# lightbulb128/troy-nova

Hardware: AMD Instinct MI355X
Metric: homomorphic mul+relinearize ops/sec (CKKS mul+relin+rescale), N=16384 (higher is better)
Workload: dtype u64; 1 GPU; CKKS N=16384, 6x50-bit coeff modulus (K=6, L=5): multiply + relinearize + rescale_to_next (BASELINE configs[2]); batch_per_gpu=1024, entry=troyn_ckks_multiply_relinearize_rescale, parallelism=batch-sharded x1, keys broadcast once (RCCL), ranks=1, slowest_rank=0

## Files before the change

### troy-nova_amd/csrc/launch.hpp

```cpp
#pragma once
#include <hip/hip_runtime.h>
#include "ntt_kernels.hpp"
#include "ntt_sizes.hpp"
#include "ksmac_kernels.hpp"
#include "behz2_kernels.hpp"

#ifndef TROYN_SMALL_LP_FACTOR
#define TROYN_SMALL_LP_FACTOR 2
#endif

namespace troyn {

inline unsigned device_cu_count() {
    static thread_local int cached_dev = -1;
    static thread_local unsigned cached = 0;
    int dev = 0;
    (void)hipGetDevice(&dev);
    if (dev != cached_dev) {
        int cus = 0;
        if (hipDeviceGetAttribute(&cus, hipDeviceAttributeMultiprocessorCount, dev) != hipSuccess || cus <= 0) cus = 256;
        cached = (unsigned)cus; cached_dev = dev;
    }
    return cached;
}
inline bool is_small_launch(size_t limb_polys) { return limb_polys * TROYN_SMALL_LP_FACTOR <= device_cu_count(); }

struct LaunchCtx {
    hipStream_t s;
    int half_mask;
    bool small_two_pass_off;
    int tensor_wgs;
};

template <class A, int PART>
struct NttUnit {
    static bool transform(unsigned log_n, const NttArgs& a, size_t limb_polys, bool inverse, const LaunchCtx& lc, u64* scratch);
    static bool small_pass(unsigned log_n, int which, const NttArgs& a, size_t limb_polys, const LaunchCtx& lc);
    static bool ks_mac(unsigned log_n, const NttArgs& a, const KeyPtrs& kp, size_t blocks, const LaunchCtx& lc);
    static bool tensor(unsigned log_n, int stage, const NttArgs& a, const NttArgs& b, const NttArgs& d, size_t batch, const LaunchCtx& lc);
};
extern template struct NttUnit<ArithF64, 1>;
extern template struct NttUnit<ArithF64, 2>;
extern template struct NttUnit<ArithU64, 1>;
extern template struct NttUnit<ArithU64, 2>;
template <class F>
inline bool in_ntt_unit(unsigned log_n, bool f64, F&& f) {
    if (ntt_part_of(log_n) == 1) return f64 ? f(NttUnit<ArithF64, 1>{}) : f(NttUnit<ArithU64, 1>{});
    return f64 ? f(NttUnit<ArithF64, 2>{}) : f(NttUnit<ArithU64, 2>{});
}

inline bool launch_transform(unsigned log_n, bool f64, const NttArgs& a, size_t limb_polys, bool inverse, const LaunchCtx& lc, u64* scratch) {
    return in_ntt_unit(log_n, f64, [&](auto u) { return decltype(u)::transform(log_n, a, limb_polys, inverse, lc, scratch); });
}
void launch_ntt_generic(const NttArgs& a, unsigned log_n, bool inverse, size_t limb_polys, const LaunchCtx& lc);
inline bool launch_small_pass(unsigned log_n, bool f64, int which, const NttArgs& a, size_t limb_polys, const LaunchCtx& lc) {
    return in_ntt_unit(log_n, f64, [&](auto u) { return decltype(u)::small_pass(log_n, which, a, limb_polys, lc); });
}
void launch_mrr_quartet(unsigned log_n, size_t batch, const NttArgs& sp, const NttArgs& la, const NttArgs& ta, hipStream_t s, bool limb_parallel);
void launch_mrr_quartet_load(unsigned log_n, size_t groups, const NttArgs& iv, const NttArgs& fw, hipStream_t s, bool f64);
void launch_mrr_tail(unsigned log_n, size_t batch, const NttArgs& sp, const NttArgs& la, const NttArgs& ta, hipStream_t s);
inline bool launch_ks_mac(unsigned log_n, bool f64, const NttArgs& a, const KeyPtrs& kp, size_t blocks, const LaunchCtx& lc) {
    return in_ntt_unit(log_n, f64, [&](auto u) { return decltype(u)::ks_mac(log_n, a, kp, blocks, lc); });
}
inline bool launch_tensor(unsigned log_n, bool f64, int stage, const NttArgs& a, const NttArgs& b, const NttArgs& d, size_t batch, const LaunchCtx& lc) {
    return in_ntt_unit(log_n, f64, [&](auto u) { return decltype(u)::tensor(log_n, stage, a, b, d, batch, lc); });
}
bool launch_tensor_accumulate(unsigned log_n, bool f64, const NttArgs& fa, const TensorAccPtrs& terms, unsigned count, const NttArgs& id, size_t batch, const LaunchCtx& lc);
void launch_ksmac2(unsigned log_n, size_t batch, unsigned rows, const KsMacArgs& a, hipStream_t s, bool digits_f64 = false, bool wide_digits = false);
void launch_ksmac2_split(unsigned log_n, size_t batch, const KsMacArgs& a, hipStream_t s, bool digits_f64, int epi);
void launch_ksmac_prepare_keys(const KeyPtrs& kp, unsigned L, unsigned polys, unsigned n, double* out, unsigned blocks, hipStream_t s,
                               const ulonglong2* scale = nullptr, const DevModulus* mods = nullptr, unsigned scale_rows = 0,
                               double* diag_out = nullptr);
struct KsMacIArgs;
void launch_ksmaci(unsigned log_n, size_t batch, const KsMacIArgs& a, hipStream_t s, int epi);
void launch_ksmaci_prepare_keys(const KeyPtrs& kp, unsigned L, unsigned K, unsigned n, unsigned long long row_mask, ulonglong2* out, unsigned blocks, hipStream_t s,
                                const ulonglong2* scale, const DevModulus* mods, unsigned scale_rows, ulonglong2* diag_out);
void launch_behz2_lift(unsigned L, bool smallq, unsigned grid, hipStream_t s, unsigned chunks, const Behz2Dev& c, const u64* src, u64* dst, bool aux50 = false);
bool launch_behz2_lift_pass1(unsigned L, size_t items, hipStream_t s, const Behz2Dev& c, const u64* src, u64* dst_q, u64* dst_bsk,
                             const double* tw_q, const double* tw_aux, const DevModulus* q_mods, const DevModulus* aux_mods);
bool launch_behz2_floor_pass2(unsigned L, size_t items, hipStream_t s, const Behz2Dev& c, const u64* in_q, const u64* in_bsk, u64* out,
                              const double* tw_q, const double* tw_aux, const DevModulus* q_mods, const DevModulus* aux_mods);
void launch_behz2_floor(unsigned L, bool smallq, unsigned grid, hipStream_t s, unsigned chunks, const Behz2Dev& c, const u64* in_q, const u64* in_bsk, u64* out, bool aux50 = false);

struct CkksFftArgs;
struct CkksComposeArgs;
bool ckks_fft_two_pass(unsigned log_n);
bool launch_ckks_fft(unsigned log_n, bool decode, const CkksFftArgs& a, size_t batch, hipStream_t s);
void launch_ckks_encode_polynomial(const double* coeffs, unsigned count, double scale, unsigned n, const DevModulus* mods, unsigned L, u64* residues,
                                   unsigned* too_large, size_t batch, hipStream_t s);
bool launch_ckks_compose(const CkksComposeArgs& a, size_t batch, hipStream_t s);
struct ModRaiseArgs;
bool launch_ckks_mod_raise(const ModRaiseArgs& a, size_t items, unsigned chunks, hipStream_t s);

}
```

### troy-nova_amd/csrc/troyn.hip

```cpp
#include <hip/hip_runtime.h>

#include <algorithm>
#include <atomic>
#include <cmath>
#include <complex>
#include <cstdio>
#include <cstdlib>
#include <cstring>
#include <functional>
#include <memory>
#include <mutex>
#include <string>
#include <vector>

#include "../../include/troyn.h"
#include "behz_kernels.hpp"
#include "behz2_kernels.hpp"
#include "launch.hpp"
#include "crypto_kernels.hpp"
#include "bgv_kernels.hpp"
#include "ring2k_kernels.hpp"
#include "host_math.hpp"
#include "ntt_kernels.hpp"
#include "ksmac_kernels.hpp"
#include "ksmaci_kernels.hpp"
#include "poly_kernels.hpp"
#include "hoist_kernels.hpp"
#include "ckks_kernels.hpp"
#include "ckks_tables.hpp"
#include "raise_kernels.hpp"

using namespace troyn;

static thread_local std::string g_last_error;

static int fail(int code, const std::string& msg) {
    g_last_error = msg;
    return code;
}

#define HIP_TRY(expr)                                                                      \
    do {                                                                                   \
        hipError_t e_ = (expr);                                                            \
        if (e_ != hipSuccess) return fail((int)e_, std::string(#expr) + ": " + hipGetErrorString(e_)); \
    } while (0)

namespace {
struct PinnedSlot { void* host = nullptr; hipEvent_t done = nullptr; };
struct PinnedRing {
    static constexpr size_t SLOTS = 8, BYTES = 256u << 10;
    PinnedSlot slot[SLOTS];
    size_t next = 0;
};
}
static int upload_host_table(hipStream_t s, void* dev, const void* host, size_t bytes) {
    if (bytes == 0) return TROYN_OK;
    int device = 0;
    HIP_TRY(hipGetDevice(&device));
    constexpr int MAX_DEVICES = 16;
    static thread_local PinnedRing* rings[MAX_DEVICES] = {};
    if (bytes > PinnedRing::BYTES || device < 0 || device >= MAX_DEVICES) {
        HIP_TRY(hipMemcpyAsync(dev, host, bytes, hipMemcpyHostToDevice, s));
        HIP_TRY(hipStreamSynchronize(s));
        return TROYN_OK;
    }
    if (!rings[device]) rings[device] = new PinnedRing;
    PinnedRing& ring = *rings[device];
    PinnedSlot& sl = ring.slot[ring.next];
    if (!sl.host) {
        hipEvent_t ev = nullptr;
        HIP_TRY(hipEventCreateWithFlags(&ev, hipEventDisableTiming));
        void* host_buf = nullptr;
        const hipError_t me = hipHostMalloc(&host_buf, PinnedRing::BYTES, hipHostMallocPortable);
        if (me != hipSuccess) { (void)hipEventDestroy(ev); return fail((int)me, std::string("hipHostMalloc: ") + hipGetErrorString(me)); }
        sl.done = ev; sl.host = host_buf;
    } else {
        HIP_TRY(hipEventSynchronize(sl.done));
    }
// ... 94 lines not shown
    return TROYN_OK;
}

extern "C" int troyn_kernel_timer_read(int region, double* total_ms, uint64_t* launches) {
    if (region < 0 || region >= TROYN_TIMER_REGIONS || !total_ms || !launches) return fail(TROYN_E_INVALID, "[troyn_kernel_timer_read] bad argument");
    std::vector<TimerSpan> spans;
    { std::lock_guard<std::mutex> g(g_ktimer.mu); spans.swap(g_ktimer.spans[region]); }
    double total = 0.0;
    hipError_t err = hipSuccess;
    int cur = -1;
    (void)hipGetDevice(&cur);
    for (auto& sp : spans) {
        if (err != hipSuccess) break;
        if (sp.device != cur) { if ((err = hipSetDevice(sp.device)) != hipSuccess) break; }
        float ms = 0.f;
        if ((err = hipEventSynchronize(sp.e1)) == hipSuccess && (err = hipEventElapsedTime(&ms, sp.e0, sp.e1)) == hipSuccess) total += ms;
        if (sp.device != cur) (void)hipSetDevice(cur);
    }
    {
        std::lock_guard<std::mutex> g(g_ktimer.mu);
        for (auto& sp : spans) g_ktimer.free_pairs.push_back(sp);
    }
    if (err != hipSuccess) return fail((int)err, std::string("[troyn_kernel_timer_read] ") + hipGetErrorString(err));
    *total_ms = total; *launches = spans.size();
    return TROYN_OK;
}

struct TroynOptions {
    bool ntt_u64 = false;
    int ntt_split = -1;
    bool tensor_split = false;
    bool tensor_fused = false;
    int ks_order = -1;
    int ks_split = -1;
    bool ks_tail_split = false;
    bool ks_mac_split = false;
    bool ks_mac_fused = false;
    bool ks_diag_loop = false;
    int ks_rows = 0;
    bool ks_mac_shoup_off = false;
    bool mrr_mixed_off = false;
    bool mrr_small_off = false;
    bool mrr_small_serial = false;
    bool mrr_calls = false;
    int mrr_chunk = 0, mrr_streams = 2;
    bool behz_v1 = false;
    bool behz_base_ref = false;
    bool behz_lift_split = false;
    int plain_mac = 0;
    int ntt_half = -1;
    bool ntt_overlap_off = false;
    bool ntt_small_two_pass_off = false;
    int tensor_wgs = 8;
};
static const char* const TROYN_OPTION_NAMES[] = {"TROYN_NTT_ARITH", "TROYN_NTT_SPLIT", "TROYN_BFV_TENSOR", "TROYN_KS_ORDER", "TROYN_KS_SPLIT", "TROYN_KS_TAIL", "TROYN_KS_MAC",
    "TROYN_KS_DIAG", "TROYN_KS_ROWS", "TROYN_KS_MAC_SHOUP", "TROYN_MRR_MIXED", "TROYN_MRR_SMALL", "TROYN_MRR", "TROYN_MRR_CHUNK", "TROYN_MRR_STREAMS", "TROYN_BEHZ", "TROYN_BEHZ_BASE", "TROYN_BEHZ_LIFT",
    "TROYN_PLAIN_MAC", "TROYN_NTT_HALF", "TROYN_NTT_SMALL_TWO_PASS", "TROYN_TENSOR_WGS", "TROYN_NTT_OVERLAP"};
static int option_apply(TroynOptions& o, const char* name, const char* value) {
    const TroynOptions d;
    const std::string n = name ? name : "", v = value ? value : "";
    bool bad = false;
    auto word = [&](std::initializer_list<const char*> words, int dflt) {
        if (v.empty()) return dflt;
        int i = 0;
        for (const char* w : words) { if (v == w) return i; i++; }
        bad = true;
        return dflt;
    };
    auto num = [&](long lo, long hi, int dflt) {
        if (v.empty()) return dflt;
        char* end = nullptr;
        const long x = strtol(v.c_str(), &end, 0);
        if (end == v.c_str() || *end || x < lo || x > hi) { bad = true; return dflt; }
        return (int)x;
    };
    TroynOptions t = o;
    if (n == "TROYN_NTT_ARITH") t.ntt_u64 = word({"auto", "u64"}, 0) == 1;
    else if (n == "TROYN_NTT_SPLIT") t.ntt_split = num(0, 1, d.ntt_split);
    else if (n == "TROYN_BFV_TENSOR") { const int w = word({"auto", "split", "fused"}, 0); t.tensor_split = w == 1; t.tensor_fused = w == 2; }
    else if (n == "TROYN_KS_ORDER") t.ks_order = word({"plain", "item", "row", "band"}, d.ks_order);
    else if (n == "TROYN_KS_SPLIT") t.ks_split = num(0, 1, d.ks_split);
    else if (n == "TROYN_KS_TAIL") t.ks_tail_split = word({"fused", "split"}, 0) == 1;
    else if (n == "TROYN_KS_MAC") { const int w = word({"auto", "split", "fused"}, 0); t.ks_mac_split = w == 1; t.ks_mac_fused = w == 2; }
    else if (n == "TROYN_KS_DIAG") t.ks_diag_loop = word({"epilogue", "loop"}, 0) == 1;
    else if (n == "TROYN_KS_ROWS") t.ks_rows = num(0, 64, d.ks_rows);
    else if (n == "TROYN_KS_MAC_SHOUP") t.ks_mac_shoup_off = num(0, 1, 1) == 0;
    else if (n == "TROYN_MRR_MIXED") t.mrr_mixed_off = num(0, 1, 1) == 0;
    else if (n == "TROYN_MRR_SMALL") { const int w = word({"1", "0", "serial"}, 0); t.mrr_small_off = w == 1; t.mrr_small_serial = w == 2; }
    else if (n == "TROYN_MRR") t.mrr_calls = word({"fused", "calls"}, 0) == 1;
    else if (n == "TROYN_MRR_CHUNK") t.mrr_chunk = num(0, 1 << 20, d.mrr_chunk);
    else if (n == "TROYN_MRR_STREAMS") t.mrr_streams = num(1, 4, d.mrr_streams);
    else if (n == "TROYN_BEHZ") t.behz_v1 = word({"v2", "v1"}, 0) == 1;
    else if (n == "TROYN_BEHZ_BASE") t.behz_base_ref = word({"small", "ref"}, 0) == 1;
    else if (n == "TROYN_BEHZ_LIFT") t.behz_lift_split = word({"fused", "split"}, 0) == 1;
    else if (n == "TROYN_PLAIN_MAC") t.plain_mac = word({"auto", "v1", "single", "dual", "quad"}, 0);
    else if (n == "TROYN_NTT_HALF") t.ntt_half = num(0, 0xffff, d.ntt_half);
    else if (n == "TROYN_NTT_SMALL_TWO_PASS") t.ntt_small_two_pass_off = num(0, 1, 1) == 0;
    else if (n == "TROYN_NTT_OVERLAP") t.ntt_overlap_off = num(0, 1, 1) == 0;
    else if (n == "TROYN_TENSOR_WGS") { t.tensor_wgs = num(2, 8, d.tensor_wgs); if (t.tensor_wgs != 8 && t.tensor_wgs != 3 && t.tensor_wgs != 2) bad = true; }
    else return 0;
    if (bad) return -1;
    o = t;
    return 1;
}
static int options_from_environment(TroynOptions& o) {
    for (const char* name : TROYN_OPTION_NAMES)
        if (const char* e = getenv(name))
            if (option_apply(o, name, e) < 0) return fail(TROYN_E_INVALID, std::string("[troyn_plan_create] environment: ") + name + "=" + e + " is not a value of this option");
    return TROYN_OK;
}

struct troyn_plan {
    int device = 0;
    TroynOptions opt;
    std::atomic<uint64_t> opt_gen{0};
    unsigned log_n = 0, n = 0, K = 0;
    std::vector<u64> moduli;
    std::vector<host::NttTable> tables;
    DevModulus* d_mods = nullptr;
    ulonglong2* d_fwd = nullptr;
    ulonglong2* d_inv = nullptr;
    double* d_fwd_f64 = nullptr;
    double* d_inv_f64 = nullptr;
    std::vector<char> small_modulus;
    ulonglong2* d_inv_last = nullptr;
    double* d_fwd_r1 = nullptr;
    double* d_fwd_r2 = nullptr;
    ulonglong2* d_fwd_r1i = nullptr;
    ulonglong2* d_fwd_r2i = nullptr;
};

static inline void select_device_index(int device) {
    int cur = -1;
    if (hipGetDevice(&cur) != hipSuccess || cur != device) (void)hipSetDevice(device);
}
static inline void select_device(const troyn_plan* p) { if (p) select_device_index(p->device); }
template <typename H> static inline void select_device(const H* h) { if (h && h->plan) select_device_index(h->plan->device); }


static DevModulus make_dev_modulus(u64 q, unsigned log_n, bool with_inv_n) {
    DevModulus m;
    std::memset(&m, 0, sizeof(m));
    m.q = q;
    host::BarrettRatio r = host::barrett_ratio(q);
    m.ratio_lo = r.lo; m.ratio_hi = r.hi;
    if (with_inv_n) {
        u64 ninv = 0;
        if (host::invmod(((u64)1 << log_n) % q, q, ninv)) {
            host::Shoup s = host::shoup(ninv, q);
            m.inv_n_op = s.operand; m.inv_n_quo = s.quotient;
            if (q < F64_MODULUS_LIMIT) { m.inv_n_d = (double)ninv; m.inv_n_pd = (double)ninv * (1.0 / (double)q); }
        }
    }
    if (q < F64_MODULUS_LIMIT) { m.pd = (double)q; m.inv_pd = 1.0 / (double)q; }
    return m;
}

static inline ulonglong2 shoup_pair(u64 w, u64 m) {
    const host::Shoup s = host::shoup(w % m, m);
    return make_ulonglong2(s.operand, s.quotient);
}

static auto element_of(const std::vector<u64>& v) { return [&v](size_t i) { return v[i]; }; }

static int inv_punctured(const std::vector<u64>& q, std::vector<u64>& out) {
    out.assign(q.size(), 1);
    for (size_t i = 0; q.size() > 1 && i < q.size(); i++)
        if (!host::invmod(host::product_mod(q, i, q[i]) % q[i], q[i], out[i])) return fail(TROYN_E_MODULUS, "[RNSBase::initialize] RNSBase product is not invertible.");
    return TROYN_OK;
}

template <typename T>
static int upload_vector(T** dev, const std::vector<T>& v) {
    HIP_TRY(hipMalloc(dev, v.size() * sizeof(T)));
    HIP_TRY(hipMemcpy(*dev, v.data(), v.size() * sizeof(T), hipMemcpyHostToDevice));
    return TROYN_OK;
}

struct ConstBlob {
    std::vector<u64> host;
    std::vector<std::function<void(const u64*)>> bound;
    std::vector<u64>& aligned() { if (host.size() & 1) host.push_back(0); return host; }
    template <typename F>
    size_t words(size_t count, F f) {
        const size_t off = host.size();
        for (size_t i = 0; i < count; i++) host.push_back(f(i));
        return off;
    }
    template <typename F, typename M>
    size_t shoup(size_t count, F f, M modulus_of) {
        const size_t off = aligned().size();
        for (size_t i = 0; i < count; i++) { const ulonglong2 s = shoup_pair(f(i), modulus_of(i)); host.push_back(s.x); host.push_back(s.y); }
        return off;
    }
    template <typename T> static const T* at(const u64* dev, size_t off) { return reinterpret_cast<const T*>(dev + off); }
    template <typename T> void bind(const T** field, size_t off) { bound.push_back([=](const u64* dev) { *field = at<T>(dev, off); }); }
    int upload(int device, u64** dev) const {
        HIP_TRY(hipSetDevice(device));
        if (int rc = upload_vector(dev, host)) return rc;
        for (const auto& set : bound) set(*dev);
        return TROYN_OK;
    }
};

template <typename T, typename Conv>
static std::vector<T> twiddle_rows(const troyn_plan* p, bool inverse, Conv conv) {
    std::vector<T> rows;
    rows.reserve((size_t)p->K * p->n);
    for (size_t i = 0; i < p->K; i++)
        for (const host::Shoup& w : inverse ? p->tables[i].inv : p->tables[i].fwd) rows.push_back(conv(i, w));
    return rows;
}

template <typename T, typename Conv>
static void round_vectors(const troyn_plan* p, Conv conv, std::vector<T>& r1, std::vector<T>& r2) {
    const size_t K = p->K, n = p->n, r1n = (n >> 10) * 32;
    r1.assign(K * r1n, conv(0, host::Shoup{0, 0}));
    r2.assign(K * n, conv(0, host::Shoup{0, 0}));
    for (size_t i = 0; i < K; i++) {
        const auto& fw = p->tables[i].fwd;
        for (unsigned s = 1; s < 32; s++) {
            unsigned lvl = 0;
            while ((2u << lvl) <= s) lvl++;
            const unsigned g = s - (1u << lvl);
            for (size_t th = 0; th < (n >> 10); th++) r1[i * r1n + th * 32 + s] = conv(i, fw[(((n >> 10) + th) << lvl) + g]);
            for (size_t T_ = 0; T_ < (n >> 5); T_++) r2[i * n + ksm_perm((unsigned)(T_ * 32 + s))] = conv(i, fw[(((n >> 5) + T_) << lvl) + g]);
        }
    }
}

static int plan_upload(troyn_plan* p) {
    const size_t K = p->K, n = p->n;
    std::vector<DevModulus> mods(K);
    p->small_modulus.assign(K, 0);
    for (size_t i = 0; i < K; i++) {
        mods[i] = make_dev_modulus(p->moduli[i], p->log_n, true);
        mods[i].inv_n_op = p->tables[i].inv_degree.operand;
        mods[i].inv_n_quo = p->tables[i].inv_degree.quotient;
        p->small_modulus[i] = p->moduli[i] < F64_MODULUS_LIMIT;
        if (p->small_modulus[i] && n >= 2) {
            const u64 nw = host::mulmod(p->tables[i].inv[n - 1].operand, p->tables[i].inv_degree.operand, p->moduli[i]);
            mods[i].inv_n_w_d = (double)nw;
            mods[i].inv_n_w_pd = (double)nw * (1.0 / (double)p->moduli[i]);
        }
    }
    std::vector<ulonglong2> inv_last((K + 1) * K, make_ulonglong2(0, 0));
    for (size_t L = 2; L <= K; L++)
        for (size_t i = 0; i + 1 < L; i++) {
            u64 inv = 0;
            if (!host::invmod(p->moduli[L - 1] % p->moduli[i], p->moduli[i], inv))
                return fail(TROYN_E_MODULUS, "[troyn_plan_create] Unable to invert q[last] mod q[i].");
            inv_last[L * K + i] = shoup_pair(inv, p->moduli[i]);
        }
    static_assert(sizeof(host::Shoup) == sizeof(ulonglong2), "Shoup layout");
    auto pair = [](size_t, const host::Shoup& w) { return make_ulonglong2(w.operand, w.quotient); };
    auto f64 = [&](size_t i, const host::Shoup& w) { return p->small_modulus[i] ? (double)w.operand : 0.0; };
    int rc;
    if ((rc = upload_vector(&p->d_mods, mods))) return rc;
    if ((rc = upload_vector(&p->d_fwd, twiddle_rows<ulonglong2>(p, false, pair)))) return rc;
    if ((rc = upload_vector(&p->d_inv, twiddle_rows<ulonglong2>(p, true, pair)))) return rc;
    if ((rc = upload_vector(&p->d_inv_last, inv_last))) return rc;
    if ((rc = upload_vector(&p->d_fwd_f64, twiddle_rows<double>(p, false, f64)))) return rc;
    if ((rc = upload_vector(&p->d_inv_f64, twiddle_rows<double>(p, true, f64)))) return rc;
    if (p->log_n >= 13 && p->log_n <= 15) {
        std::vector<double> r1, r2;
        round_vectors(p, f64, r1, r2);
        if ((rc = upload_vector(&p->d_fwd_r1, r1)) || (rc = upload_vector(&p->d_fwd_r2, r2))) return rc;
        std::vector<ulonglong2> r1i, r2i;
        round_vectors(p, pair, r1i, r2i);
        if ((rc = upload_vector(&p->d_fwd_r1i, r1i)) || (rc = upload_vector(&p->d_fwd_r2i, r2i))) return rc;
    }
    return TROYN_OK;
}

static void plan_free(troyn_plan* p) {
    if (!p) return;
    if (p->d_mods) (void)hipFree(p->d_mods);
    if (p->d_fwd) (void)hipFree(p->d_fwd);
    if (p->d_inv) (void)hipFree(p->d_inv);
    if (p->d_inv_last) (void)hipFree(p->d_inv_last);
    if (p->d_fwd_f64) (void)hipFree(p->d_fwd_f64);
    if (p->d_inv_f64) (void)hipFree(p->d_inv_f64);
    if (p->d_fwd_r1) (void)hipFree(p->d_fwd_r1);
    if (p->d_fwd_r2) (void)hipFree(p->d_fwd_r2);
    if (p->d_fwd_r1i) (void)hipFree(p->d_fwd_r1i);
    if (p->d_fwd_r2i) (void)hipFree(p->d_fwd_r2i);
    delete p;
}

extern "C" int troyn_plan_create(troyn_plan** plan, int device, uint32_t log_n, uint32_t n_moduli,
                                 const uint64_t* moduli, const uint64_t* roots) {
    if (!plan || !moduli) return fail(TROYN_E_INVALID, "[troyn_plan_create] null argument");
    *plan = nullptr;
    if (log_n < 1 || log_n > 17) return fail(TROYN_E_INVALID, "[troyn_plan_create] Invalid poly_modulus_degree.");
    if (n_moduli < 1 || n_moduli > 64) return fail(TROYN_E_INVALID, "[troyn_plan_create] Invalid coeff modulus count.");
    std::unique_ptr<troyn_plan, void (*)(troyn_plan*)> p(new troyn_plan, plan_free);
    p->device = device; p->log_n = log_n; p->n = 1u << log_n; p->K = n_moduli;
    { const int orc = options_from_environment(p->opt); if (orc != TROYN_OK) return orc; }
    p->moduli.assign(moduli, moduli + n_moduli);
    for (uint32_t i = 0; i < n_moduli; i++) {
        u64 q = moduli[i];
        if ((q >> 61) != 0 || q < 2) return fail(TROYN_E_MODULUS, "[Modulus::set_value] Value can be at most 61-bit and cannot be 1.");
        for (uint32_t j = 0; j < i; j++)
            if (moduli[j] == q) return fail(TROYN_E_MODULUS, "[troyn_plan_create] coeff_modulus must be pairwise coprime.");
        try {
            p->tables.push_back(host::make_ntt_table(log_n, q, roots ? roots[i] : 0));
        } catch (const std::exception& e) {
            return fail(TROYN_E_MODULUS, e.what());
        }
    }
    HIP_TRY(hipSetDevice(device));
    int rc = plan_upload(p.get());
    if (rc != TROYN_OK) return rc;
    *plan = p.release();
    return TROYN_OK;
}

extern "C" int troyn_plan_destroy(troyn_plan* plan) {
    plan_free(plan);
    return TROYN_OK;
}

extern "C" int troyn_plan_set_option(troyn_plan* plan, const char* name, const char* value) {
    if (!plan || !name) return fail(TROYN_E_INVALID, "[troyn_plan_set_option] null argument");
    const int rc = option_apply(plan->opt, name, value);
    if (rc == 0) return fail(TROYN_E_INVALID, std::string("[troyn_plan_set_option] unknown option ") + name);
    if (rc < 0) return fail(TROYN_E_INVALID, std::string("[troyn_plan_set_option] ") + name + "=" + value + " is not a value of this option");
    plan->opt_gen.fetch_add(1, std::memory_order_release);
    return TROYN_OK;
}

extern "C" uint32_t troyn_plan_log_n(const troyn_plan* plan) { return plan ? plan->log_n : 0; }
extern "C" uint32_t troyn_plan_n_moduli(const troyn_plan* plan) { return plan ? plan->K : 0; }

extern "C" int troyn_plan_get_root(const troyn_plan* plan, uint32_t mi, uint64_t* root) {
    select_device(plan);
    if (!plan || !root || mi >= plan->K) return fail(TROYN_E_INVALID, "[troyn_plan_get_root] bad argument");
    *root = plan->tables[mi].root;
    return TROYN_OK;
// ... 1474 lines not shown
    return w;
}

constexpr int MRR_MAX_STREAMS = 4;
struct MrrStreams { hipStream_t s[MRR_MAX_STREAMS] = {}; hipEvent_t fork = nullptr, join[MRR_MAX_STREAMS] = {}; int device = -1; };
static MrrStreams* mrr_streams(int device) {
    static thread_local std::vector<MrrStreams> pool;
    for (auto& m : pool) if (m.device == device) return &m;
    MrrStreams m;
    m.device = device;
    bool ok = true;
    for (int q = 0; q < MRR_MAX_STREAMS && ok; q++) {
        ok = hipStreamCreateWithFlags(&m.s[q], hipStreamNonBlocking) == hipSuccess;
        ok = ok && hipEventCreateWithFlags(&m.join[q], hipEventDisableTiming) == hipSuccess;
    }
    ok = ok && hipEventCreateWithFlags(&m.fork, hipEventDisableTiming) == hipSuccess;
    if (!ok) {
        for (int q = 0; q < MRR_MAX_STREAMS; q++) {
            if (m.join[q]) (void)hipEventDestroy(m.join[q]);
            if (m.s[q]) (void)hipStreamDestroy(m.s[q]);
        }
        if (m.fork) (void)hipEventDestroy(m.fork);
        return nullptr;
    }
    pool.push_back(m);
    return &pool.back();
}

static bool ksmac_no_load_corr_ok(const troyn_plan* p, unsigned L) {
    if (p->log_n != 14 || p->opt.ntt_u64) return false;
    double qmax = 0.0;
    for (unsigned j = 0; j < L; j++) qmax = std::max(qmax, (double)p->moduli[j]);
    for (unsigned k = 0; k <= L; k++) {
        const double pm = (double)p->moduli[k == L ? p->K - 1 : k];
        double a = qmax + 0.875 * pm;
        for (int layer = 0; layer < 3; layer++) a += (0.5 + 1.5 * a * 0x1p-52) * pm;
        if (!(a < 0.98 * 0x1p53)) return false;
    }
    return true;
}

struct MrrCall {
    const troyn_plan* p; uint32_t L; const u64* a; const u64* b; u64* out; u64* ws; const MrrLayout& w; size_t batch; hipStream_t s;
    bool all_f64, special_wide, last_wide;
    unsigned t_flags() const { return (special_wide ? NTT_FLAG_TS_U64 : 0u) | (last_wide ? NTT_FLAG_TL_U64 : 0u); }
    long long ct_b() const { return 2ll * L * p->n; }
    long long ct_p() const { return (long long)L * p->n; }
    u64* poly_prod() const { return ws + w.poly_prod; }
    template <typename F> int for_runs(unsigned count, unsigned polys, F&& f) const {
        return for_class_runs(p, 0, count, class_by_policy, !all_f64 && batch * (size_t)polys * count >= OVERLAP_MIN_LIMB_POLYS, s, f);
    }
};

static int mrr_digits(const MrrCall& c) {
    const troyn_plan* p = c.p; const unsigned L = c.L, n = p->n;
    return c.for_runs(L, 1, [&](unsigned j0, unsigned j1, hipStream_t rs) {
        NttArgs x = contiguous_args(p, c.a + (size_t)j0 * n, c.ws + c.w.digits + (size_t)j0 * n, 1, j1 - j0, j0, j1 - j0, TROYN_IDX_COMPONENTWISE, 0);
        x.in_bstride = c.ct_b(); x.in_pstride = c.ct_p();
        x.out_bstride = (long long)L * n; x.out_pstride = (long long)L * n;
        x.mul_a = c.a; x.mul_b = c.b; x.mul_bstride = c.ct_b(); x.mul_pstride = c.ct_p(); x.mul_limb0 = j0;
        x.fused_mode = NTT_FUSED_MULPAIR;
        if (c.all_f64) x.flags = NTT_FLAG_STORE_F64;
        return launch_ntt(p, x, c.batch, true, rs);
    });
}

static int mrr_inner_product(const MrrCall& c, const KsRows& rows, const double* kf, const ulonglong2* ki, const KeyPtrs* raw) {
    const troyn_plan* p = c.p; const unsigned L = c.L, K = p->K, n = p->n;
    TimerScope ts(TROYN_TIMER_KS_INNER_PRODUCT, c.s);
    if (rows.small) {
        KsMacArgs m = ksmac2_args(p, L, c.batch, c.ws + c.w.digits, (long long)L * n, c.poly_prod(), kf);
        m.diag = c.a + c.ct_p(); m.diag_b = c.b + c.ct_p(); m.diag_bstride = c.ct_b(); m.diag_cstride = n;
        m.ten_a = c.a; m.ten_b = c.b; m.ten_bstride = c.ct_b(); m.ten_pstride = c.ct_p();
        m.diag_keys = kf + (size_t)L * 2 * K * n;
        if (rows.wide) m.row_mask = rows.small;
        m.no_load_corr = (c.all_f64 && ksmac_no_load_corr_ok(p, L)) ? 1u : 0u;
        if (raw) {
            m.grouped = 0;
            m.part = reinterpret_cast<double*>(c.ws + c.w.split); m.part_jstride = (long long)c.batch * m.out_bstride;
            m.split_skip_diag = 1;
            m.raw = *raw; m.raw_pstride = (long long)K * n; m.split_scale = p->d_inv_last + (size_t)K * K;
            launch_ksmac2_split(p->log_n, c.batch, m, c.s, true, 1);
        } else launch_ksmac2(p->log_n, c.batch, (unsigned)__builtin_popcountll(rows.small), m, c.s, c.all_f64, rows.wide_digits);
        LAUNCH_CHECK();
    }
    if (rows.wide) {
        KsMacIArgs m = ksmaci_args(p, L, c.batch, c.ws + c.w.digits, (long long)L * n, c.poly_prod(), ki, rows.wide);
        m.ten_a = c.a; m.ten_b = c.b; m.ten_bstride = c.ct_b(); m.ten_pstride = c.ct_p();
        launch_ksmaci(p->log_n, c.batch, m, c.s, 2);
        LAUNCH_CHECK();
    }
    return TROYN_OK;
}

static NttArgs mrr_last_args(const MrrCall& c) {
    const troyn_plan* p = c.p; const unsigned L = c.L, K = p->K, n = p->n;
    NttArgs x = contiguous_args(p, c.poly_prod() + (size_t)(L - 1) * n, c.ws + c.w.last_intt, 2, 1, L - 1, 1, TROYN_IDX_COMPONENTWISE, 0);
    x.in_pstride = (long long)(L + 1) * n; x.in_bstride = 2ll * (L + 1) * n;
    x.in2 = c.ws + c.w.spec_intt; x.in2_bstride = 2ll * n; x.in2_pstride = n;
    x.aux_mod = K - 1; x.inv_table = p->d_inv_last + (size_t)K * K + (L - 1);
    x.fused_mode = (!c.last_wide && c.special_wide) ? NTT_FUSED_LAST_LIMB_W : NTT_FUSED_LAST_LIMB;
    x.flags = c.t_flags();
    return x;
}
static NttArgs mrr_tail_args(const MrrCall& c, unsigned j0, unsigned j1) {
    const troyn_plan* p = c.p; const unsigned L = c.L, K = p->K, n = p->n;
    NttArgs x = contiguous_args(p, c.ws + c.w.spec_intt, c.out + (size_t)j0 * n, 2, j1 - j0, j0, j1 - j0, TROYN_IDX_COMPONENTWISE, 0);
    x.in_bstride = 2ll * n; x.in_pstride = n; x.in_cstride = 0;
    x.out_bstride = 2ll * (L - 1) * n; x.out_pstride = (long long)(L - 1) * n;
    x.in2 = c.ws + c.w.last_intt; x.in2_bstride = 2ll * n; x.in2_pstride = n;
    x.aux_mod = K - 1; x.inv_table = p->d_inv_last + (size_t)K * K + j0;
    x.aux2_mod = L - 1; x.inv_table2 = p->d_inv_last + (size_t)L * K + j0;
    x.ext0 = c.poly_prod() + (size_t)j0 * n; x.ext0_bstride = 2ll * (L + 1) * n; x.ext0_pstride = (long long)(L + 1) * n; x.ext0_cstride = n;
    x.fused_mode = (class_by_policy(p, j0) && c.t_flags()) ? NTT_FUSED_TAIL_RESCALE_W : NTT_FUSED_TAIL_RESCALE;
    x.flags = c.t_flags();
    return x;
}

static int mrr_tail_merged(const MrrCall& c, bool quartet) {
    const troyn_plan* p = c.p; const unsigned L = c.L, K = p->K, n = p->n;
    const LaunchCtx lc = launch_ctx(p, c.s);
    if (quartet) {
        u64* rows = c.poly_prod() + (size_t)(L - 1) * n;
        NttArgs pa = contiguous_args(p, rows, rows, 2, 2, L - 1, K - (L - 1), TROYN_IDX_KS_SKIP_FINALS, 1);
        pa.in_pstride = pa.out_pstride = (long long)(L + 1) * n; pa.in_bstride = pa.out_bstride = 2ll * (L + 1) * n;
        prep_direct(p, pa, true, true);
        launch_small_pass(p->log_n, true, 0, pa, c.batch * 4, lc);
        LAUNCH_CHECK();
    }
    NttArgs sp = special_rows_args(p, c.poly_prod(), nullptr, L);
    prep_direct(p, sp, true, true);
    NttArgs la = mrr_last_args(c);
    prep_direct(p, la, true, true);
    NttArgs ta = mrr_tail_args(c, 0, L - 1);
    prep_direct(p, ta, true, false);
    if (!quartet) {
        launch_mrr_tail(p->log_n, c.batch, sp, la, ta, c.s);
        LAUNCH_CHECK();
        return TROYN_OK;
    }
    launch_mrr_quartet(p->log_n, c.batch, sp, la, ta, c.s, !p->opt.mrr_small_serial && is_small_launch(c.batch * 2 * (size_t)(L - 1)));
    LAUNCH_CHECK();
    as_input_of(ta, ta);
    ta.reduce_input = 0;
    launch_small_pass(p->log_n, true, 1, ta, c.batch * 2 * (L - 1), lc);
    LAUNCH_CHECK();
    return TROYN_OK;
}

static int mrr_chain(const troyn_plan* p, uint32_t L, const KsRows& rows, const u64* a, const u64* b, const double* kf, const ulonglong2* ki, u64* out, u64* ws,
                     const MrrLayout& w, size_t batch, hipStream_t s, const KeyPtrs* raw = nullptr) {
    const MrrCall c{p, L, a, b, out, ws, w, batch, s, mrr_all_f64(p, L), !class_by_policy(p, p->K - 1), !class_by_policy(p, L - 1)};
    int rc;
    if ((rc = mrr_digits(c))) return rc;
    if ((rc = mrr_inner_product(c, rows, kf, ki, raw))) return rc;
    if (c.all_f64 && (small_tail_wanted(p, batch * 2 * (size_t)(L - 1)) || (p->log_n == 15 && !p->opt.mrr_small_off))) return mrr_tail_merged(c, true);
    if (c.all_f64 && p->log_n == 14 && !p->opt.mrr_small_off) return mrr_tail_merged(c, false);
    {
        NttArgs x = special_rows_args(p, c.poly_prod(), ws + w.spec_intt, L);
        x.flags = NTT_FLAG_STORE_ROUND_HALF;
        if ((rc = launch_ntt(p, x, batch, true, s))) return rc;
    }
    if ((rc = launch_ntt(p, mrr_last_args(c), batch, true, s))) return rc;
    return c.for_runs(L - 1, 2, [&](unsigned j0, unsigned j1, hipStream_t rs) { return launch_ntt(p, mrr_tail_args(c, j0, j1), batch, false, rs); });
}

extern "C" size_t troyn_ckks_multiply_relinearize_rescale_workspace_bytes(const troyn_plan* plan, uint32_t L, size_t batch) {
    if (!plan || L < 2 || L > plan->K) return 0;
    return mrr_layout(plan, L, batch).total * sizeof(u64);
}

extern "C" int troyn_ckks_multiply_relinearize_rescale(const troyn_plan* p, uint32_t L, const uint64_t* a_, const uint64_t* b_,
                                                       const uint64_t* const* keys, uint64_t* out_, void* workspace, size_t workspace_bytes,
                                                       size_t batch, troyn_stream_t stream) {
    select_device(p);
    const char* P = "[troyn_ckks_multiply_relinearize_rescale]";
    if (!p || !a_ || !b_ || !keys || !out_ || !workspace) return fail(TROYN_E_INVALID, std::string(P) + " null argument");
    const unsigned K = p->K, n = p->n;
    if (K < 2) return fail(TROYN_E_INVALID, "[Evaluator::switch_key_inplace_internal] Keyswitching is not supported.");
    if (L < 2 || L > K - 1) return fail(TROYN_E_INVALID, "[Evaluator::mod_switch_scale_to_next_internal] Next context data is not set.");
    const MrrLayout w = mrr_layout(p, L, batch);
    if (workspace_bytes < w.total * sizeof(u64)) return fail(TROYN_E_WORKSPACE, std::string(P) + " workspace too small");
    if (batch == 0) return TROYN_OK;
    hipStream_t s = (hipStream_t)stream;
    const u64* a = (const u64*)a_; const u64* b = (const u64*)b_;
    u64* out = (u64*)out_;
    u64* ws = (u64*)workspace;
    int rc;
    const bool unfused = p->opt.mrr_calls;
    if (!mrr_fast_path(p, L) || unfused || ks_small_mixed(p, L, batch) || batch * (size_t)(L + 1) * 4 > 0x7fffffffull) {
        if ((rc = launch_convolute(p->d_mods, n, 0, L, a, 2, b, 2, ws + w.prod3, batch, s))) return rc;
        const size_t sub_bytes = (w.total - w.sub) * sizeof(u64);
        if ((rc = troyn_relinearize(p, L, 1, 1, (const uint64_t*)(ws + w.prod3), keys, (uint64_t*)(ws + w.relin2), ws + w.sub, sub_bytes, batch, stream))) return rc;
        return troyn_divide_and_round_q_last_ntt(p, L, (const uint64_t*)(ws + w.relin2), 2, out_, ws + w.sub, sub_bytes, batch, stream);
    }
    KeyPtrs kp;
    std::memset(&kp, 0, sizeof(kp));
    for (unsigned j = 0; j < L; j++) {
        if (!keys[j]) return fail(TROYN_E_INVALID, "[Evaluator::switch_key_inplace_internal] null key pointer");
        kp.p[j] = (const u64*)keys[j];
    }
    const int chunk_env = p->opt.mrr_chunk;
    size_t chunk = batch;
    if (chunk_env > 0 && batch >= 2 * (size_t)chunk_env && (chunk_env % 8) == 0) chunk = (size_t)chunk_env;
    const bool all_f64 = mrr_all_f64(p, L);
    const bool split = chunk == batch && all_f64 && ksmac_split_wanted(p, batch, L, p->log_n);
    double* kf = reinterpret_cast<double*>(ws + w.keys_f64);
    ulonglong2* ki = reinterpret_cast<ulonglong2*>(ws + w.keys_int);
    const KsRows rows = ks_rows(p, L);
    if (!split && rows.small && (rc = prepare_keys_f64(p, kp, L, kf, L, true, s))) return rc;
// ... 1617 lines not shown
```

Baseline: 304,500 ops/s.

## Add dedicated fused mulpair + inverse NTT kernel for N=16384 digit decomposition

Adds a specialized kernel that multiplies the c1 components of both ciphertexts and performs the inverse NTT per limb in one workgroup. It uses register-resident radix-32 rounds, LDS transposes and precomputed per-round inverse twiddle tables uploaded at plan creation, and writes f64 digits directly. This replaces the generic NTT launch with its fused MULPAIR mode in the digit step whenever the whole-limb MRR path applies. The intent is to cut global memory passes and launch overhead. In exchange the plan holds extra twiddle tables and there is a large hand-scheduled kernel specific to log_n=14.

After: 311,300 ops/s, median of 6. 2.2% higher.

```diff
diff --git a/troy-nova_amd/csrc/launch.hpp b/troy-nova_amd/csrc/launch.hpp
--- a/troy-nova_amd/csrc/launch.hpp
+++ b/troy-nova_amd/csrc/launch.hpp
@@ -59,6 +59,8 @@
 void launch_mrr_quartet(unsigned log_n, size_t batch, const NttArgs& sp, const NttArgs& la, const NttArgs& ta, hipStream_t s, bool limb_parallel);
 void launch_mrr_quartet_load(unsigned log_n, size_t groups, const NttArgs& iv, const NttArgs& fw, hipStream_t s, bool f64);
 void launch_mrr_tail(unsigned log_n, size_t batch, const NttArgs& sp, const NttArgs& la, const NttArgs& ta, hipStream_t s);
+struct MulpairHalfArgs;
+bool launch_mulpair_half(unsigned log_n, size_t batch, const MulpairHalfArgs& a, hipStream_t s);
 inline bool launch_ks_mac(unsigned log_n, bool f64, const NttArgs& a, const KeyPtrs& kp, size_t blocks, const LaunchCtx& lc) {
     return in_ntt_unit(log_n, f64, [&](auto u) { return decltype(u)::ks_mac(log_n, a, kp, blocks, lc); });
 }
diff --git a/troy-nova_amd/csrc/mulpair_half_kernels.hpp b/troy-nova_amd/csrc/mulpair_half_kernels.hpp
--- /dev/null
+++ b/troy-nova_amd/csrc/mulpair_half_kernels.hpp
@@ -0,0 +1,175 @@
+#pragma once
+#include "ksmac_kernels.hpp"
+
+#ifndef MPH_LOAD_WINDOW
+#define MPH_LOAD_WINDOW 8
+#endif
+
+namespace troyn {
+
+struct MulpairHalfArgs {
+    const u64* a1; const u64* b1;
+    long long in_bstride;
+    u64* out; long long out_bstride;
+    const DevModulus* mods;
+    const double* tw;
+    const double* tw_r1;
+    const double* tw_r2;
+    unsigned L;
+    unsigned store_f64;
+};
+
+template <int RB, int G0, int NG, bool FIX>
+__device__ __forceinline__ void mph_layer(double (&x)[32], const double* tw, const F64Mod& fm) {
+    static_for<0, NG>([&](auto gc) {
+        constexpr int g = G0 + decltype(gc)::value;
+        const double w = tw[decltype(gc)::value];
+        static_for<0, (1 << RB)>([&](auto oc) {
+            constexpr int R0 = (g << (RB + 1)) | decltype(oc)::value, R1 = R0 | (1 << RB);
+            const double u = x[R0], v = x[R1];
+            x[R0] = FIX ? f64_corr(u + v, fm) : u + v;
+            x[R1] = f64_mulq(u - v, w, fm.inv_p, fm.p);
+        });
+    });
+}
+
+template <class LD>
+__device__ __forceinline__ void mph_round5(double (&x)[32], double (&ta)[8], double (&tb)[8], LD&& ld, const F64Mod& fm) {
+    mph_layer<0, 0, 8, false>(x, ta, fm);
+    __builtin_amdgcn_sched_barrier(0);
+    static_for<0, 4>([&](auto qc) { const double2 v = ld(4 + decltype(qc)::value); ta[2 * decltype(qc)::value] = v.x; ta[2 * decltype(qc)::value + 1] = v.y; });
+    mph_layer<0, 8, 8, false>(x, tb, fm);
+    __builtin_amdgcn_sched_barrier(0);
+    static_for<0, 4>([&](auto qc) { const double2 v = ld(decltype(qc)::value); tb[2 * decltype(qc)::value] = v.x; tb[2 * decltype(qc)::value + 1] = v.y; });
+    mph_layer<1, 0, 8, true>(x, ta, fm);
+    __builtin_amdgcn_sched_barrier(0);
+    mph_layer<2, 0, 4, false>(x, tb + 4, fm);
+    mph_layer<3, 0, 2, true>(x, tb + 2, fm);
+    mph_layer<4, 0, 1, false>(x, tb + 1, fm);
+    __builtin_amdgcn_sched_barrier(0);
+}
+
+template <int W>
+__global__ __launch_bounds__(KSM_THREADS, 2) void mulpair_half_kernel(MulpairHalfArgs a) {
+    constexpr unsigned N = 1u << 14, HW = 1u << KSM_TB;
+    static_assert(W >= 1 && W <= 16, "load window: 1..16 register pairs");
+    __shared__ __attribute__((aligned(16))) u64 lds[KSM_LDS_WORDS];
+
+    const unsigned t = threadIdx.x, lane = t & 63u, wave = t >> 6;
+    const unsigned j = blockIdx.x % a.L, b = blockIdx.x / a.L;
+    const ArithF64::Mod md = ArithF64::make(a.mods[j]);
+    const F64Mod fm = md.m;
+
+    typedef const double __attribute__((address_space(4)))* cdp;
+    const cdp tws = (cdp)(unsigned long long)(a.tw + (size_t)j * N);
+    const double* r1b = a.tw_r1 + (size_t)j * (N >> 10) * 32;
+    const double* r2b = a.tw_r2 + (size_t)j * N;
+    const unsigned r1off = (t >> 5) * 256u, slice_off = wave * 16384u + lane * 16u;
+
+    const unsigned p0 = ksm_phys(t << 1);
+    const unsigned p1 = ksm_phys((t & 31u) | ((t >> 5) << 10));
+    const unsigned p2 = ksm_phys(t << 5);
+    const unsigned pt = ksm_phys(wave * 2048u + lane * 2u);
+
+    const u64* ga = a.a1 + (long long)b * a.in_bstride + (size_t)j * N;
+    const u64* gb = a.b1 + (long long)b * a.in_bstride + (size_t)j * N;
+
+    ulonglong2 va[16], vb[16];
+    auto request = [&](auto hc, auto ic) {
+        constexpr int h = decltype(hc)::value, m = decltype(ic)::value;
+        va[m] = ksm_gload<ulonglong2>(ksm_uniform(ga + h * HW) + m * 128, slice_off);
+        vb[m] = ksm_gload<ulonglong2>(ksm_uniform(gb + h * HW) + m * 128, slice_off);
+    };
+
+    auto front = [&](auto hc, double (&x)[32]) {
+        constexpr int h = decltype(hc)::value;
+        const double* r1u = ksm_uniform(r1b + h * ((KSM_THREADS >> 5) * 32));
+        const double* r2u = ksm_uniform(r2b + h * HW);
+        double ta[8], tb[8];
+        static_for<0, 4>([&](auto qc) { constexpr int q = decltype(qc)::value; const double2 v = ksm_gload<double2>(r2u + 128 * (8 + q), slice_off); ta[2 * q] = v.x; ta[2 * q + 1] = v.y; });
+        static_for<0, 4>([&](auto qc) { constexpr int q = decltype(qc)::value; const double2 v = ksm_gload<double2>(r2u + 128 * (12 + q), slice_off); tb[2 * q] = v.x; tb[2 * q + 1] = v.y; });
+        static_for<0, 16>([&](auto mc) {
+            constexpr int m = decltype(mc)::value;
+            __builtin_amdgcn_sched_barrier(0);
+            const double2 pr = make_double2(f64_mulq(f64_from_u64(va[m].x), f64_from_u64(vb[m].x), fm.inv_p, fm.p),
+                                            f64_mulq(f64_from_u64(va[m].y), f64_from_u64(vb[m].y), fm.inv_p, fm.p));
+            *reinterpret_cast<double2*>(&lds[pt + ksm_phys(m * 128u)]) = pr;
+            __builtin_amdgcn_sched_barrier(0);
+            if constexpr (m + W < 16) request(hc, std::integral_constant<int, m + W>{});
+        });
+        __builtin_amdgcn_wave_barrier();
+        static_for<0, 16>([&](auto mc) {
+            constexpr int m = decltype(mc)::value;
+            const double2 v = *reinterpret_cast<const double2*>(&lds[p2 + 2 * m]);
+            x[2 * m] = v.x; x[2 * m + 1] = v.y;
+        });
+        __builtin_amdgcn_sched_barrier(0);
+        mph_round5(x, ta, tb, [&](int q) { return ksm_gload<double2>(r2u + 128 * q, slice_off); }, fm);
+        static_for<0, 16>([&](auto mc) {
+            constexpr int m = decltype(mc)::value;
+            *reinterpret_cast<double2*>(&lds[p2 + 2 * m]) = make_double2(f64_corr(x[2 * m], fm), f64_corr(x[2 * m + 1], fm));
+        });
+        static_for<0, 4>([&](auto qc) { constexpr int q = decltype(qc)::value; const double2 v = ksm_gload<double2>(r1u + 2 * (8 + q), r1off); ta[2 * q] = v.x; ta[2 * q + 1] = v.y; });
+        static_for<0, 4>([&](auto qc) { constexpr int q = decltype(qc)::value; const double2 v = ksm_gload<double2>(r1u + 2 * (12 + q), r1off); tb[2 * q] = v.x; tb[2 * q + 1] = v.y; });
+        __builtin_amdgcn_wave_barrier();
+        static_for<0, 32>([&](auto rc) {
+            constexpr int R = decltype(rc)::value;
+            x[R] = f64_bits_to_double(lds[p1 + 34 * R]);
+        });
+        __builtin_amdgcn_sched_barrier(0);
+        mph_round5(x, ta, tb, [&](int q) { return ksm_gload<double2>(r1u + 2 * q, r1off); }, fm);
+        static_for<0, 32>([&](auto rc) {
+            constexpr int R = decltype(rc)::value;
+            lds[p1 + 34 * R] = f64_double_to_bits(f64_corr(x[R], fm));
+        });
+        __syncthreads();
+        static_for<0, 16>([&](auto ic) {
+            constexpr int i = decltype(ic)::value;
+            constexpr unsigned off = ksm_phys(((i & 1) << 9) | ((i >> 1) << 10));
+            const double2 v = *reinterpret_cast<const double2*>(&lds[p0 + off]);
+            x[2 * i] = v.x; x[2 * i + 1] = v.y;
+        });
+        __builtin_amdgcn_sched_barrier(0);
+    };
+    auto round_c = [&](auto hc, double (&x)[32]) {
+        constexpr unsigned h = decltype(hc)::value;
+        static_for<0, 3>([&](auto lc) {
+            constexpr int li = decltype(lc)::value;
+            constexpr int bit = 10 + li, rb = bit - 8, l = 13 - bit;
+            constexpr int NG = 1 << (12 - bit);
+            double w[NG];
+            static_for<0, NG>([&](auto gc) { constexpr unsigned g = decltype(gc)::value; w[g] = tws[N - (2u << l) + 1u + (h << (12 - bit)) + g]; });
+            mph_layer<rb, 0, NG, li == 1>(x, w, fm);
+        });
+        __builtin_amdgcn_sched_barrier(0);
+    };
+
+    double x0[32], x1[32];
+    const std::integral_constant<int, 0> H0{};
+    const std::integral_constant<int, 1> H1{};
+    __builtin_amdgcn_sched_barrier(0);
+    static_for<0, W>([&](auto ic) { request(H0, ic); });
+    front(H0, x0);
+    static_for<0, W>([&](auto ic) { request(H1, ic); });
+    __builtin_amdgcn_sched_barrier(0);
+    round_c(H0, x0);
+    __syncthreads();
+    front(H1, x1);
+    round_c(H1, x1);
+
+    const bool digits_f64 = a.store_f64 != 0;
+    const double dg_add = digits_f64 ? 0.0 : F64_TWO52;
+    const unsigned dg_mask_hi = digits_f64 ? 0xffffffffu : 0x000fffffu;
+    u64* go = ksm_uniform(a.out + (long long)b * a.out_bstride + (size_t)j * N);
+    static_for<0, 16>([&](auto ic) {
+        constexpr int i = decltype(ic)::value;
+        constexpr unsigned woff = ((i & 1) << 9) + ((i >> 1) << 10);
+        double s0 = x0[2 * i], d0 = x1[2 * i], s1 = x0[2 * i + 1], d1 = x1[2 * i + 1];
+        ArithF64::inv_fold(s0, d0, md);
+        ArithF64::inv_fold(s1, d1, md);
+        nt_store2_at(go + woff, t << 4, ArithF64::digit_word(s0, false, dg_add, dg_mask_hi, md), ArithF64::digit_word(s1, false, dg_add, dg_mask_hi, md));
+        nt_store2_at(go + HW + woff, t << 4, ArithF64::digit_word(d0, true, dg_add, dg_mask_hi, md), ArithF64::digit_word(d1, true, dg_add, dg_mask_hi, md));
+    });
+}
+
+}
diff --git a/troy-nova_amd/csrc/troyn.hip b/troy-nova_amd/csrc/troyn.hip
--- a/troy-nova_amd/csrc/troyn.hip
+++ b/troy-nova_amd/csrc/troyn.hip
@@ -24,6 +24,7 @@
 #include "ntt_kernels.hpp"
 #include "ksmac_kernels.hpp"
 #include "ksmaci_kernels.hpp"
+#include "mulpair_half_kernels.hpp"
 #include "poly_kernels.hpp"
 #include "hoist_kernels.hpp"
 #include "ckks_kernels.hpp"
@@ -224,10 +225,11 @@
     bool ntt_overlap_off = false;
     bool ntt_small_two_pass_off = false;
     int tensor_wgs = 8;
+    bool mulpair_half_off = false;
 };
 static const char* const TROYN_OPTION_NAMES[] = {"TROYN_NTT_ARITH", "TROYN_NTT_SPLIT", "TROYN_BFV_TENSOR", "TROYN_KS_ORDER", "TROYN_KS_SPLIT", "TROYN_KS_TAIL", "TROYN_KS_MAC",
     "TROYN_KS_DIAG", "TROYN_KS_ROWS", "TROYN_KS_MAC_SHOUP", "TROYN_MRR_MIXED", "TROYN_MRR_SMALL", "TROYN_MRR", "TROYN_MRR_CHUNK", "TROYN_MRR_STREAMS", "TROYN_BEHZ", "TROYN_BEHZ_BASE", "TROYN_BEHZ_LIFT",
-    "TROYN_PLAIN_MAC", "TROYN_NTT_HALF", "TROYN_NTT_SMALL_TWO_PASS", "TROYN_TENSOR_WGS", "TROYN_NTT_OVERLAP"};
+    "TROYN_PLAIN_MAC", "TROYN_NTT_HALF", "TROYN_NTT_SMALL_TWO_PASS", "TROYN_TENSOR_WGS", "TROYN_NTT_OVERLAP", "TROYN_MULPAIR_HALF"};
 static int option_apply(TroynOptions& o, const char* name, const char* value) {
     const TroynOptions d;
     const std::string n = name ? name : "", v = value ? value : "";
@@ -269,6 +271,7 @@
     else if (n == "TROYN_NTT_HALF") t.ntt_half = num(0, 0xffff, d.ntt_half);
     else if (n == "TROYN_NTT_SMALL_TWO_PASS") t.ntt_small_two_pass_off = num(0, 1, 1) == 0;
     else if (n == "TROYN_NTT_OVERLAP") t.ntt_overlap_off = num(0, 1, 1) == 0;
+    else if (n == "TROYN_MULPAIR_HALF") t.mulpair_half_off = num(0, 1, 1) == 0;
     else if (n == "TROYN_TENSOR_WGS") { t.tensor_wgs = num(2, 8, d.tensor_wgs); if (t.tensor_wgs != 8 && t.tensor_wgs != 3 && t.tensor_wgs != 2) bad = true; }
     else return 0;
     if (bad) return -1;
@@ -300,6 +303,8 @@
     double* d_fwd_r2 = nullptr;
     ulonglong2* d_fwd_r1i = nullptr;
     ulonglong2* d_fwd_r2i = nullptr;
+    double* d_inv_r1 = nullptr;
+    double* d_inv_r2 = nullptr;
 };
 
 static inline void select_device_index(int device) {
@@ -397,6 +402,23 @@
             const unsigned g = s - (1u << lvl);
             for (size_t th = 0; th < (n >> 10); th++) r1[i * r1n + th * 32 + s] = conv(i, fw[(((n >> 10) + th) << lvl) + g]);
             for (size_t T_ = 0; T_ < (n >> 5); T_++) r2[i * n + ksm_perm((unsigned)(T_ * 32 + s))] = conv(i, fw[(((n >> 5) + T_) << lvl) + g]);
+        }
+    }
+}
+
+template <typename T, typename Conv>
+static void inverse_round_vectors(const troyn_plan* p, Conv conv, std::vector<T>& r1, std::vector<T>& r2) {
+    const size_t K = p->K, n = p->n, r1n = (n >> 10) * 32;
+    r1.assign(K * r1n, conv(0, host::Shoup{0, 0}));
+    r2.assign(K * n, conv(0, host::Shoup{0, 0}));
+    for (size_t i = 0; i < K; i++) {
+        const auto& iv = p->tables[i].inv;
+        for (unsigned s = 1; s < 32; s++) {
+            unsigned lvl = 0;
+            while ((2u << lvl) <= s) lvl++;
+            const unsigned g = s - (1u << lvl);
+            for (size_t th = 0; th < (n >> 10); th++) r1[i * r1n + th * 32 + s] = conv(i, iv[n - ((n >> 9) << lvl) + 1 + (th << lvl) + g]);
+            for (size_t T_ = 0; T_ < (n >> 5); T_++) r2[i * n + ksm_perm((unsigned)(T_ * 32 + s))] = conv(i, iv[n - ((n >> 4) << lvl) + 1 + (T_ << lvl) + g]);
         }
     }
 }
@@ -442,6 +464,11 @@
         round_vectors(p, pair, r1i, r2i);
         if ((rc = upload_vector(&p->d_fwd_r1i, r1i)) || (rc = upload_vector(&p->d_fwd_r2i, r2i))) return rc;
     }
+    if (p->log_n == 14) {
+        std::vector<double> r1, r2;
+        inverse_round_vectors(p, f64, r1, r2);
+        if ((rc = upload_vector(&p->d_inv_r1, r1)) || (rc = upload_vector(&p->d_inv_r2, r2))) return rc;
+    }
     return TROYN_OK;
 }
 
@@ -457,6 +484,8 @@
     if (p->d_fwd_r2) (void)hipFree(p->d_fwd_r2);
     if (p->d_fwd_r1i) (void)hipFree(p->d_fwd_r1i);
     if (p->d_fwd_r2i) (void)hipFree(p->d_fwd_r2i);
+    if (p->d_inv_r1) (void)hipFree(p->d_inv_r1);
+    if (p->d_inv_r2) (void)hipFree(p->d_inv_r2);
     delete p;
 }
 
@@ -2037,8 +2066,23 @@
     }
 };
 
+static bool mrr_whole_limb_class(const MrrCall& c) {
+    const troyn_plan* p = c.p;
+    return c.all_f64 && p->log_n == 14 && !p->opt.mrr_small_off && !small_tail_wanted(p, c.batch * 2 * (size_t)(c.L - 1));
+}
+
 static int mrr_digits(const MrrCall& c) {
     const troyn_plan* p = c.p; const unsigned L = c.L, n = p->n;
+    if (mrr_whole_limb_class(c) && !p->opt.mulpair_half_off && p->d_inv_r2) {
+        MulpairHalfArgs x;
+        x.a1 = c.a + c.ct_p(); x.b1 = c.b + c.ct_p(); x.in_bstride = c.ct_b();
+        x.out = c.ws + c.w.digits; x.out_bstride = (long long)L * n;
+        x.mods = p->d_mods; x.tw = p->d_inv_f64; x.tw_r1 = p->d_inv_r1; x.tw_r2 = p->d_inv_r2;
+        x.L = L; x.store_f64 = 1u;
+        if (!launch_mulpair_half(p->log_n, c.batch, x, c.s)) return fail(TROYN_E_INVALID, "[troyn_ckks_multiply_relinearize_rescale] batch too large for one launch");
+        LAUNCH_CHECK();
+        return TROYN_OK;
+    }
     return c.for_runs(L, 1, [&](unsigned j0, unsigned j1, hipStream_t rs) {
         NttArgs x = contiguous_args(p, c.a + (size_t)j0 * n, c.ws + c.w.digits + (size_t)j0 * n, 1, j1 - j0, j0, j1 - j0, TROYN_IDX_COMPONENTWISE, 0);
         x.in_bstride = c.ct_b(); x.in_pstride = c.ct_p();
@@ -2140,7 +2184,7 @@
     if ((rc = mrr_digits(c))) return rc;
     if ((rc = mrr_inner_product(c, rows, kf, ki, raw))) return rc;
     if (c.all_f64 && (small_tail_wanted(p, batch * 2 * (size_t)(L - 1)) || (p->log_n == 15 && !p->opt.mrr_small_off))) return mrr_tail_merged(c, true);
-    if (c.all_f64 && p->log_n == 14 && !p->opt.mrr_small_off) return mrr_tail_merged(c, false);
+    if (mrr_whole_limb_class(c)) return mrr_tail_merged(c, false);
     {
         NttArgs x = special_rows_args(p, c.poly_prod(), ws + w.spec_intt, L);
         x.flags = NTT_FLAG_STORE_ROUND_HALF;
diff --git a/troy-nova_amd/csrc/troyn_mulpair_half.hip b/troy-nova_amd/csrc/troyn_mulpair_half.hip
--- /dev/null
+++ b/troy-nova_amd/csrc/troyn_mulpair_half.hip
@@ -0,0 +1,12 @@
+#include "launch.hpp"
+#include "mulpair_half_kernels.hpp"
+
+namespace troyn {
+
+bool launch_mulpair_half(unsigned log_n, size_t batch, const MulpairHalfArgs& a, hipStream_t s) {
+    if (log_n != 14 || batch * a.L == 0 || batch * a.L > 0x7fffffffull) return false;
+    hipLaunchKernelGGL(mulpair_half_kernel<MPH_LOAD_WINDOW>, dim3((unsigned)(batch * a.L)), dim3(KSM_THREADS), 0, s, a);
+    return true;
+}
+
+}
```
